# darksim33/Pyneapple

Hardware: AMD Instinct MI355X
Metric: voxels/sec (pixelwise triexp LM & 250-bin NNLS) at 1/2/4/8 MI355X (higher is better)
Workload: dtype f64

## Files before the change

### pyneapple_amd/csrc/pnx_curvefit_kernel.hpp

```cpp
#pragma once
#include <hip/hip_runtime.h>
#include <stdint.h>

namespace pnx {

constexpr int kWave = 64;
constexpr int kMaxB = 128;
constexpr int kMaxP = 8;
#ifdef PNX_ROW_BLK
template <int N> constexpr int row_blk() { return PNX_ROW_BLK; }
#else
template <int N> constexpr int row_blk() { return N >= 7 ? 2 : (N >= 5 ? 4 : 8); }
#endif
constexpr double kEps = 2.220446049250313e-16;
constexpr double kSqrtEps = 1.4901161193847656e-08;
typedef __attribute__((address_space(3))) void lds_void;

struct StreamCtl {
    unsigned long long ready;
    unsigned int abort;
    unsigned int timed_out;
    unsigned int done[1];
};

struct CurvefitArgs {
    const double *y;
    const double *p0;
    const double *lo;
    const double *hi;
    const double *fixed;
    double *popt;
    double *pcov;
    int8_t *status;
    int32_t *nfev;
    double *cost;
    unsigned long long *queue;
    const int32_t *order;
    StreamCtl *ctl;
    unsigned int *host_flags;
    int granule_shift;
    unsigned int stream_spins;
    int phase;
    long long n_vox;
    int n_b;
    int per_voxel;
    int fixed_per_voxel;
    int max_nfev;
    int n_fixed;
    int t1_mode;
    double tr, tm;
    double ftol, xtol, gtol;
    double p0s[kMaxP], los[kMaxP], his[kMaxP], fixeds[kMaxP];
    int free_idx[kMaxP];
    int fixed_idx[kMaxP];
    int use_sigma;
    int absolute_sigma;
    double b[kMaxB];
    double w[kMaxB];
};

template <int MODEL> struct Model;

template <> struct Model<0> {
    static constexpr int NALL = 2, NC = 1;
    __device__ static constexpr int dpos(int c) { return 1; }
    __device__ static double signal(const double *p, const double *E) { return p[0] * E[0]; }
    __device__ static void jac(const double *p, const double *E, double x, double *r) {
        r[0] = E[0];
        r[1] = -x * p[0] * E[0];
    }
};
template <> struct Model<1> {
    static constexpr int NALL = 3, NC = 2;
    __device__ static constexpr int dpos(int c) { return c == 0 ? 1 : 2; }
    __device__ static double signal(const double *p, const double *E) { return p[0] * E[0] + (1 - p[0]) * E[1]; }
    __device__ static void jac(const double *p, const double *E, double x, double *r) {
        r[0] = E[0] - E[1];
        r[1] = -x * p[0] * E[0];
        r[2] = -x * (1 - p[0]) * E[1];
    }
};
template <> struct Model<2> {
    static constexpr int NALL = 4, NC = 2;
    __device__ static constexpr int dpos(int c) { return c == 0 ? 1 : 2; }
    __device__ static double signal(const double *p, const double *E) {
        return p[3] * (p[0] * E[0] + (1 - p[0]) * E[1]);
    }
    __device__ static void jac(const double *p, const double *E, double x, double *r) {
        r[0] = p[3] * (E[0] - E[1]);
        r[1] = -x * p[3] * p[0] * E[0];
        r[2] = -x * p[3] * (1 - p[0]) * E[1];
        r[3] = p[0] * E[0] + (1 - p[0]) * E[1];
    }
};
template <> struct Model<3> {
    static constexpr int NALL = 4, NC = 2;
    __device__ static constexpr int dpos(int c) { return c == 0 ? 1 : 3; }
    __device__ static double signal(const double *p, const double *E) { return p[0] * E[0] + p[2] * E[1]; }
    __device__ static void jac(const double *p, const double *E, double x, double *r) {
        r[0] = E[0];
        r[1] = -x * p[0] * E[0];
        r[2] = E[1];
        r[3] = -x * p[2] * E[1];
    }
};
template <> struct Model<4> {
    static constexpr int NALL = 5, NC = 3;
    __device__ static constexpr int dpos(int c) { return c == 0 ? 1 : (c == 1 ? 3 : 4); }
    __device__ static double signal(const double *p, const double *E) {
        return p[0] * E[0] + p[2] * E[1] + (1 - p[0] - p[2]) * E[2];
    }
    __device__ static void jac(const double *p, const double *E, double x, double *r) {
        const double f3 = 1 - p[0] - p[2];
        r[0] = E[0] - E[2];
        r[1] = -x * p[0] * E[0];
        r[2] = E[1] - E[2];
        r[3] = -x * p[2] * E[1];
        r[4] = -x * f3 * E[2];
    }
};
template <> struct Model<5> {
    static constexpr int NALL = 6, NC = 3;
    __device__ static constexpr int dpos(int c) { return c == 0 ? 1 : (c == 1 ? 3 : 4); }
    __device__ static double signal(const double *p, const double *E) {
        return p[5] * (p[0] * E[0] + p[2] * E[1] + (1 - p[0] - p[2]) * E[2]);
    }
    __device__ static void jac(const double *p, const double *E, double x, double *r) {
        const double f3 = 1 - p[0] - p[2], S0 = p[5];
        r[0] = S0 * (E[0] - E[2]);
        r[1] = -x * S0 * p[0] * E[0];
        r[2] = S0 * (E[1] - E[2]);
        r[3] = -x * S0 * p[2] * E[1];
        r[4] = -x * S0 * f3 * E[2];
        r[5] = p[0] * E[0] + p[2] * E[1] + f3 * E[2];
    }
};
template <> struct Model<6> {
    static constexpr int NALL = 6, NC = 3;
    __device__ static constexpr int dpos(int c) { return c == 0 ? 1 : (c == 1 ? 3 : 5); }
    __device__ static double signal(const double *p, const double *E) {
        return p[0] * E[0] + p[2] * E[1] + p[4] * E[2];
    }
    __device__ static void jac(const double *p, const double *E, double x, double *r) {
        r[0] = E[0];
        r[1] = -x * p[0] * E[0];
        r[2] = E[1];
        r[3] = -x * p[2] * E[1];
        r[4] = E[2];
        r[5] = -x * p[4] * E[2];
    }
};

template <int MODEL> __host__ __device__ constexpr int colperm(int k) {
    constexpr int P[7][6] = {{0, 1, 2, 3, 4, 5}, {2, 0, 1, 3, 4, 5}, {2, 0, 1, 3, 4, 5}, {3, 1, 2, 0, 4, 5},
                             {4, 3, 0, 2, 1, 5}, {4, 3, 0, 2, 1, 5}, {5, 3, 1, 4, 2, 0}};
    return P[MODEL][k];
}

template <int MODEL> __device__ constexpr int comp_of_param(int j) {
    for (int c = 0; c < Model<MODEL>::NC; ++c)
        if (Model<MODEL>::dpos(c) == j) return c;
    return -1;
}

template <int N> __device__ inline double dotn(const double *a, const double *b) {
    double s = 0;
#pragma unroll
    for (int i = 0; i < N; ++i) s += a[i] * b[i];
    return s;
}
template <int N> __device__ inline double normn(const double *a) { return sqrt(dotn<N>(a, a)); }

__device__ inline double fast_rcp(double x) {
    double r = __builtin_amdgcn_rcp(x);
    r = fma(fma(-x, r, 1.0), r, r);
    r = fma(fma(-x, r, 1.0), r, r);
    return r;
}
__device__ inline double fast_sqrt_rsqrt(double x, double *rs) {
    double y = __builtin_amdgcn_rsq(x);
    double g = x * y, h = 0.5 * y;
    double r = fma(-h, g, 0.5);
    g = fma(g, r, g);
    h = fma(h, r, h);
    r = fma(-h, g, 0.5);
    g = fma(g, r, g);
    h = fma(h, r, h);
    *rs = h + h;
    return g;
}

#ifndef PNX_CF_FAST_EXP
#define PNX_CF_FAST_EXP 1
#endif
#ifndef PNX_CF_HINTS
#define PNX_CF_HINTS 1
#endif
#if PNX_CF_HINTS
#define PNX_LIKELY(x) __builtin_expect(!!(x), 1)
#else
#define PNX_LIKELY(x) (x)
#endif
__device__ inline double exp_fast(double x) {
#if PNX_CF_FAST_EXP
    const double k = __builtin_rint(x * 1.4426950408889634);
    double r = fma(k, -0.6931471805599453, x);
    r = fma(k, -2.3190468138462996e-17, r);
    const double r2 = r * r;
    double qe = 2.7630903490112654e-07;
    qe = fma(qe, r2, 2.480149103909504e-05);
    qe = fma(qe, r2, 0.0013888888945916382);
    qe = fma(qe, r2, 0.041666666666519754);
    qe = fma(qe, r2, 0.5000000000000012);
    double qo = 2.502232256764614e-08;
    qo = fma(qo, r2, 2.755751454582531e-06);
    qo = fma(qo, r2, 0.00019841269589115522);
    qo = fma(qo, r2, 0.008333333333455043);
    qo = fma(qo, r2, 0.16666666666666477);
    const double q = fma(r, qo, qe);
    return ldexp(fma(r, fma(r, q, 1.0), 1.0), __double2int_rz(k));
#else
    return exp(x);
#endif
}

template <int N, int RB> __device__ inline void qr_merge(double (&R)[N][N], double (&q)[N], double (&blk)[RB][N + 1]) {
#pragma unroll
    for (int k = 0; k < N; ++k) {
        double sig = 0;
#pragma unroll
        for (int r = 0; r < RB; ++r) sig += blk[r][k] * blk[r][k];
        if (sig > 0) {
            const double alpha = R[k][k];
            double rs;
            const double nrm = fast_sqrt_rsqrt(alpha * alpha + sig, &rs);
            const double beta = alpha <= 0 ? nrm : -nrm;
            const double v0 = alpha - beta;
            const double inv_v0 = copysign(fast_rcp(fabs(v0)), v0);
            const double tau = -v0 * (alpha <= 0 ? rs : -rs);
#pragma unroll
            for (int r = 0; r < RB; ++r) blk[r][k] *= inv_v0;
            R[k][k] = beta;
#pragma unroll
            for (int j = k + 1; j <= N; ++j) {
                double w = (j < N) ? R[k][j] : q[k];
#pragma unroll
                for (int r = 0; r < RB; ++r) w += blk[r][k] * blk[r][j];
                w *= tau;
                if (j < N)
                    R[k][j] -= w;
                else
                    q[k] -= w;
#pragma unroll
                for (int r = 0; r < RB; ++r) blk[r][j] -= w * blk[r][k];
            }
        }
    }
}

template <int N> __device__ inline void jacobi_svd(double (&W)[N][N], double (&V)[N][N]) {
#pragma unroll
    for (int i = 0; i < N; ++i)
#pragma unroll
        for (int j = 0; j < N; ++j) V[i][j] = (i == j) ? 1.0 : 0.0;
    if (N == 1) return;
    for (int sweep = 0; sweep < 30; ++sweep) {
        bool rotated = false;
#pragma unroll
        for (int p = 0; p < N - 1; ++p) {
#pragma unroll
            for (int q = p + 1; q < N; ++q) {
                double a = 0, b = 0, g = 0;
#pragma unroll
                for (int i = 0; i < N; ++i) {
                    a += W[i][p] * W[i][p];
                    b += W[i][q] * W[i][q];
                    g += W[i][p] * W[i][q];
                }
                const double g2 = g * g, ab = a * b;
                if (g2 > 1.0e-30 * ab) {
                    rotated = rotated || (g2 >= 1.0e-16 * ab);
                    const double num = b - a, den = 2.0 * g;
                    double rs;
                    const double hyp = fast_sqrt_rsqrt(num * num + den * den, &rs);
                    double t = fabs(den) * fast_rcp(fabs(num) + hyp);
                    t = ((num < 0) != (den < 0)) ? -t : t;
                    double c;
                    (void)fast_sqrt_rsqrt(1.0 + t * t, &c);
                    const double s = c * t;
#pragma unroll
                    for (int i = 0; i < N; ++i) {
                        const double wp = W[i][p], wq = W[i][q];
                        W[i][p] = c * wp - s * wq;
                        W[i][q] = s * wp + c * wq;
                        const double vp = V[i][p], vq = V[i][q];
                        V[i][p] = c * vp - s * vq;
                        V[i][q] = s * vp + c * vq;
                    }
                }
            }
        }
        if (!rotated) break;
    }
}

__device__ inline double strictly_feasible0(double x, double lb, double ub) {
    if (x <= lb) x = nextafter(lb, ub);
    if (x >= ub) x = nextafter(ub, lb);
    if (x < lb || x > ub) x = 0.5 * (lb + ub);
    return x;
}
__device__ inline double strictly_feasible_r(double x, double lb, double ub) {
    const double rstep = 1e-10;
    const double lower_dist = x - lb, upper_dist = ub - x;
    const double lt = rstep * fmax(1.0, fabs(lb)), ut = rstep * fmax(1.0, fabs(ub));
    int active = 0;
    if (isfinite(lb) && lower_dist <= fmin(upper_dist, lt)) active = -1;
    if (isfinite(ub) && upper_dist <= fmin(lower_dist, ut)) active = 1;
    if (active == -1) x = lb + lt;
    if (active == 1) x = ub - ut;
    if (x < lb || x > ub) x = 0.5 * (lb + ub);
    return x;
}

template <int N>
__device__ inline double step_size_to_bound(const double *x, const double *s, const double *lb, const double *ub,
                                            int *hits) {
    double steps[N];
    double mn = INFINITY;
#pragma unroll
    for (int i = 0; i < N; ++i) {
        const double num = (s[i] > 0) ? (ub[i] - x[i]) : (lb[i] - x[i]);
        steps[i] = (s[i] != 0) ? num / s[i] : INFINITY;
        mn = fmin(mn, steps[i]);
    }
    if (hits) {
#pragma unroll
        for (int i = 0; i < N; ++i) hits[i] = (steps[i] == mn) ? ((s[i] > 0) - (s[i] < 0)) : 0;
    }
    return mn;
}

template <int N> __device__ inline void rmul(const double (&R)[N][N], const double *s, double *out) {
#pragma unroll
    for (int i = 0; i < N; ++i) {
        double a = 0;
#pragma unroll
        for (int j = i; j < N; ++j) a += R[i][j] * s[j];
        out[i] = a;
    }
}

__device__ inline double minimize_quadratic_1d(double a, double b, double lb, double ub, double c, double &y) {
    double tb = lb, yb = lb * (a * lb + b) + c;
    const double yu = ub * (a * ub + b) + c;
    if (yu < yb) {
        yb = yu;
        tb = ub;
    }
    if (a != 0) {
        const double ext = -0.5 * b / a;
        if (lb < ext && ext < ub) {
            const double ye = ext * (a * ext + b) + c;
            if (ye < yb) {
                yb = ye;
                tb = ext;
            }
        }
    }
    y = yb;
    return tb;
}

template <int N>
__device__ inline double solve_lsq_trust_region(int m, const double *uf, const double *s, const double (&V)[N][N],
                                                double smax, double smin, double Delta, double initial_alpha,
                                                double *p) {
    double suf[N], t[N];
#pragma unroll
    for (int i = 0; i < N; ++i) suf[i] = s[i] * uf[i];
    const bool full_rank = (m >= N) && (smin > kEps * m * smax);
    if (full_rank) {
#pragma unroll
        for (int i = 0; i < N; ++i) t[i] = uf[i] / s[i];
#pragma unroll
        for (int i = 0; i < N; ++i) {
            double a = 0;
#pragma unroll
            for (int k = 0; k < N; ++k) a += V[i][k] * t[k];
            p[i] = -a;
        }
        if (normn<N>(p) <= Delta) return 0.0;
    }
    double alpha_upper = normn<N>(suf) / Delta;
    double alpha_lower = 0.0;
    auto phi_and_derivative = [&](double alpha, double &phi, double &phi_prime) {
        double pn2 = 0, sp = 0;
#pragma unroll
        for (int i = 0; i < N; ++i) {
            const double denom = s[i] * s[i] + alpha;
            const double q = suf[i] / denom;
            pn2 += q * q;
            sp += suf[i] * suf[i] / (denom * denom * denom);
        }
        const double p_norm = sqrt(pn2);
        phi = p_norm - Delta;
        phi_prime = -sp / p_norm;
    };
    double phi, phi_prime;
    if (full_rank) {
        phi_and_derivative(0.0, phi, phi_prime);
        alpha_lower = -phi / phi_prime;
    }
    double alpha;
    if (!full_rank && initial_alpha == 0)
        alpha = fmax(0.001 * alpha_upper, sqrt(alpha_lower * alpha_upper));
    else
        alpha = initial_alpha;
    for (int it = 0; it < 10; ++it) {
        if (alpha < alpha_lower || alpha > alpha_upper)
            alpha = fmax(0.001 * alpha_upper, sqrt(alpha_lower * alpha_upper));
        phi_and_derivative(alpha, phi, phi_prime);
        if (phi < 0) alpha_upper = alpha;
        const double ratio = phi / phi_prime;
        alpha_lower = fmax(alpha_lower, alpha - ratio);
        alpha -= (phi + Delta) * ratio / Delta;
        if (fabs(phi) < 0.01 * Delta) break;
    }
#pragma unroll
    for (int i = 0; i < N; ++i) t[i] = suf[i] / (s[i] * s[i] + alpha);
#pragma unroll
    for (int i = 0; i < N; ++i) {
        double a = 0;
#pragma unroll
        for (int k = 0; k < N; ++k) a += V[i][k] * t[k];
        p[i] = -a;
    }
    const double sc = Delta / normn<N>(p);
#pragma unroll
    for (int i = 0; i < N; ++i) p[i] *= sc;
    return alpha;
}

template <int N>
__device__ inline double select_step(const double *x, const double (&R2)[N][N], const double *g_h, double *p,
                                     double *p_h, const double *d, double Delta, const double *lb, const double *ub,
                                     double theta, double *step, double *step_h) {
    bool inb = true;
#pragma unroll
    for (int i = 0; i < N; ++i) {
        const double xp = x[i] + p[i];
        inb = inb && (xp >= lb[i]) && (xp <= ub[i]);
    }
    double t1[N], t2[N];
    if (inb) {
        rmul<N>(R2, p_h, t1);
        const double p_value = 0.5 * dotn<N>(t1, t1) + dotn<N>(p_h, g_h);
#pragma unroll
        for (int i = 0; i < N; ++i) {
            step[i] = p[i];
            step_h[i] = p_h[i];
        }
        return -p_value;
    }
    int hits[N];
    const double p_stride = step_size_to_bound<N>(x, p, lb, ub, hits);
    double r_h[N], r[N], xb[N];
#pragma unroll
    for (int i = 0; i < N; ++i) {
        r_h[i] = hits[i] ? -p_h[i] : p_h[i];
        r[i] = d[i] * r_h[i];
    }
#pragma unroll
    for (int i = 0; i < N; ++i) {
        p[i] *= p_stride;
        p_h[i] *= p_stride;
        xb[i] = x[i] + p[i];
    }
    double to_tr;
    {
        const double a = dotn<N>(r_h, r_h), b = dotn<N>(p_h, r_h), c = dotn<N>(p_h, p_h) - Delta * Delta;
        const double dd = sqrt(b * b - a * c);
        const double q = -(b + copysign(dd, b));
        const double ta = q / a, tb = c / q;
        to_tr = fmax(ta, tb);
    }
    double to_bound = step_size_to_bound<N>(xb, r, lb, ub, nullptr);
    double r_stride = fmin(to_bound, to_tr);
    double r_stride_l, r_stride_u;
    if (r_stride > 0) {
        r_stride_l = (1 - theta) * p_stride / r_stride;
        r_stride_u = (r_stride == to_bound) ? theta * to_bound : to_tr;
    } else {
        r_stride_l = 0;
        r_stride_u = -1;
    }
    double r_value;
    if (r_stride_l <= r_stride_u) {
        rmul<N>(R2, r_h, t1);
        rmul<N>(R2, p_h, t2);
        const double a = 0.5 * dotn<N>(t1, t1);
        const double b = dotn<N>(g_h, r_h) + dotn<N>(t2, t1);
        const double c = 0.5 * dotn<N>(t2, t2) + dotn<N>(g_h, p_h);
        r_stride = minimize_quadratic_1d(a, b, r_stride_l, r_stride_u, c, r_value);
#pragma unroll
        for (int i = 0; i < N; ++i) {
            r_h[i] = r_h[i] * r_stride + p_h[i];
            r[i] = r_h[i] * d[i];
        }
    } else
        r_value = INFINITY;
#pragma unroll
    for (int i = 0; i < N; ++i) {
        p[i] *= theta;
        p_h[i] *= theta;
    }
    rmul<N>(R2, p_h, t1);
    const double p_value = 0.5 * dotn<N>(t1, t1) + dotn<N>(p_h, g_h);

    double ag_h[N], ag[N];
#pragma unroll
    for (int i = 0; i < N; ++i) {
        ag_h[i] = -g_h[i];
        ag[i] = d[i] * ag_h[i];
    }
    to_tr = Delta / normn<N>(ag_h);
    to_bound = step_size_to_bound<N>(x, ag, lb, ub, nullptr);
    double ag_stride = (to_bound < to_tr) ? theta * to_bound : to_tr;
    double ag_value;
    {
        rmul<N>(R2, ag_h, t1);
        const double a = 0.5 * dotn<N>(t1, t1);
        const double b = dotn<N>(g_h, ag_h);
        ag_stride = minimize_quadratic_1d(a, b, 0.0, ag_stride, 0.0, ag_value);
    }
    if (p_value < r_value && p_value < ag_value) {
#pragma unroll
        for (int i = 0; i < N; ++i) {
            step[i] = p[i];
            step_h[i] = p_h[i];
        }
        return -p_value;
    } else if (r_value < p_value && r_value < ag_value) {
#pragma unroll
        for (int i = 0; i < N; ++i) {
            step[i] = r[i];
            step_h[i] = r_h[i];
        }
        return -r_value;
    } else {
#pragma unroll
        for (int i = 0; i < N; ++i) {
            step[i] = ag[i] * ag_stride;
            step_h[i] = ag_h[i] * ag_stride;
        }
        return -ag_value;
    }
}

enum LaneState : int { ST_IDLE = 0, ST_INIT = 1, ST_RUN = 2, ST_FINAL = 3 };

template <int N> struct Park {
    static constexpr int NR = N * (N + 1) / 2;
    static constexpr bool kParkV = (N <= 5);
    static constexpr int NV = kParkV ? N * N : 0;
    __host__ __device__ static constexpr int per_wave(int n_b) { return kWave * (((n_b + 1) & ~1) + NR + NV); }
};

#ifndef PNX_CF_WAVES_PER_SIMD
#define PNX_CF_WAVES_PER_SIMD 1
#endif
#ifndef PNX_CF_BLOCK_WAVES
#define PNX_CF_BLOCK_WAVES 4
#endif
template <int MODEL, int N, bool FD, bool PV, bool T1, bool STREAM = false>
__global__ void __launch_bounds__(64 * PNX_CF_BLOCK_WAVES, PNX_CF_WAVES_PER_SIMD) curvefit_kernel(const CurvefitArgs A) {
    using M = Model<MODEL>;
    using PK = Park<N>;
    constexpr int NALL = M::NALL;
    constexpr int NP = NALL + (T1 ? 1 : 0);
    constexpr int NC = M::NC;
    constexpr bool HASFIXED = (N != NP);
    static_assert(!(FD && HASFIXED), "finite-difference mode is only built without fixed parameters");
    auto CP = [](int k) constexpr { return (HASFIXED || k >= NALL) ? k : colperm<MODEL>(k); };

    extern __shared__ double smem[];
    const int n_b = A.n_b;
    double *bsh = smem;
    const int lane = threadIdx.x & (kWave - 1);
    const int wave = threadIdx.x / kWave;
    const bool use_w = A.use_sigma != 0;
    const double *wsh = smem + kMaxB;
    double *ytile = smem + (use_w ? 2 * kMaxB : kMaxB) + (size_t)wave * PK::per_wave(n_b);
    double *ysh = ytile + 2 * lane;
    double *rpark = ytile + (size_t)((n_b + 1) & ~1) * kWave + lane;
    double *vpark = rpark + (size_t)PK::NR * kWave;
    for (int i = threadIdx.x; i < n_b; i += blockDim.x) bsh[i] = A.b[i];
    if (use_w)
        for (int i = threadIdx.x; i < n_b; i += blockDim.x) smem[kMaxB + i] = A.w[i];
    __syncthreads();
    const bool dma_ok = ((reinterpret_cast<uintptr_t>(A.y) & 7) == 0);

    int state = ST_IDLE;
    long long vox = -1;
    unsigned long long ready_seen = 0;
    int pub = 0;
    auto publish = [&](bool all) {
        const int n_gran = (int)((A.n_vox + (1ll << A.granule_shift) - 1) >> A.granule_shift);
        int upto = pub;
        while (upto < n_gran && (all || !__ballot(state != ST_IDLE && (vox >> A.granule_shift) <= upto))) ++upto;
        if (upto == pub) return;
        __builtin_amdgcn_fence(__ATOMIC_RELEASE, "");
        const unsigned int n_waves = gridDim.x * (blockDim.x / kWave);
        if ((threadIdx.x & (kWave - 1)) == __ffsll((unsigned long long)__ballot(1)) - 1) {
            for (int g = pub; g < upto; ++g) {
                const unsigned int old = __hip_atomic_fetch_add(&A.ctl->done[g], 1u, __ATOMIC_ACQ_REL, __HIP_MEMORY_SCOPE_SYSTEM);
                if (old + 1 == n_waves) __hip_atomic_store(&A.host_flags[g], 1u, __ATOMIC_RELEASE, __HIP_MEMORY_SCOPE_SYSTEM);
            }
        }
        pub = upto;
    };
    double x[N], lb[N], ub[N];
    double pfull[NP];
    double g[N];
    double s[N], uf[N], R2[N][N], d[N], g_h[N];
    double Vreg[PK::kParkV ? 1 : N][PK::kParkV ? 1 : N];
    double smax = 0, smin = 0, theta = 0;
    double cost = 0, Delta = 0, alpha = 0;
    int nfev = 0, term = -99;
    bool first = false;
    double xn[N], step_h_norm = 0, step_norm = 0, predicted = 0;
    if (!PV) {
#pragma unroll
        for (int k = 0; k < N; ++k) {
            lb[k] = A.los[k];
            ub[k] = A.his[k];
        }
    }

#ifdef PNX_CF_STAMP
    unsigned long long seg[8] = {0, 0, 0, 0, 0, 0, 0, 0}, act[8] = {0, 0, 0, 0, 0, 0, 0, 0}, cnt[8] = {0, 0, 0, 0, 0, 0, 0, 0};
    unsigned long long tl = __builtin_amdgcn_s_memtime();
#define CFSTAMP(k) do { __builtin_amdgcn_s_waitcnt(0); const unsigned long long t_ = __builtin_amdgcn_s_memtime(); seg[k] += t_ - tl; tl = t_; } while (0)
#define CFACT(k, cond) do { act[k] += __popcll(__ballot(cond)); cnt[k] += 1; } while (0)
#else
#define CFSTAMP(k) do {} while (0)
#define CFACT(k, cond) do {} while (0)
#endif
    auto refill = [&]() {
    while (state == ST_IDLE) {
        const unsigned long long idx = atomicAdd(A.queue, 1ULL);
        if (idx >= (unsigned long long)A.n_vox) break;
        if constexpr (STREAM) {
            if (idx >= ready_seen) {
                bool got = false;
                const unsigned int *abort_word = A.host_flags + ((A.n_vox + (1ll << A.granule_shift) - 1) >> A.granule_shift);
                for (unsigned int spins = 0; spins < A.stream_spins; ++spins) {
                    ready_seen = __hip_atomic_load(&A.ctl->ready, __ATOMIC_ACQUIRE, __HIP_MEMORY_SCOPE_SYSTEM);
                    if (idx < ready_seen) {
                        got = true;
                        break;
                    }
                    if ((spins & 15u) == 15u && __hip_atomic_load(abort_word, __ATOMIC_RELAXED, __HIP_MEMORY_SCOPE_SYSTEM)) break;
                    __builtin_amdgcn_s_sleep(127);
                }
                if (!got) {
                    if (!__hip_atomic_load(abort_word, __ATOMIC_RELAXED, __HIP_MEMORY_SCOPE_SYSTEM))
                        __hip_atomic_store(&A.ctl->timed_out, 1u, __ATOMIC_RELAXED, __HIP_MEMORY_SCOPE_SYSTEM);
                    break;
                }
            }
        }
        vox = (long long)idx;
        if constexpr (!STREAM) {
            if (A.order) vox = A.order[idx];
        }
        const double *yv = A.y + (size_t)vox * n_b;
        if (dma_ok) {
            const int pairs = n_b >> 1;
            for (int c = 0; c < pairs; ++c)
                __builtin_amdgcn_global_load_lds((const void *)(yv + 2 * c), (lds_void *)(ytile + c * 2 * kWave), 16, 0, 0);
            if (n_b & 1) {
                if (vox + 1 < A.n_vox)
                    __builtin_amdgcn_global_load_lds((const void *)(yv + n_b - 1), (lds_void *)(ytile + pairs * 2 * kWave), 16, 0, 0);
                else
                    ysh[pairs * 2 * kWave] = yv[n_b - 1];
            }
        } else {
            for (int i = 0; i < n_b; ++i) ysh[(i >> 1) * 2 * kWave + (i & 1)] = yv[i];
        }
        bool okb = true, okp = true;
        double p0v[N];
#pragma unroll
        for (int k = 0; k < N; ++k) {
            if (PV) {
                p0v[k] = A.p0[(size_t)k * A.n_vox + vox];
                lb[k] = A.lo[(size_t)k * A.n_vox + vox];
                ub[k] = A.hi[(size_t)k * A.n_vox + vox];
            } else
                p0v[k] = A.p0s[k];
            okb = okb && (lb[k] < ub[k]);
            okp = okp && (p0v[k] >= lb[k]) && (p0v[k] <= ub[k]);
        }
        if (HASFIXED) {
#pragma unroll
            for (int j = 0; j < NP; ++j) pfull[j] = 0;
            for (int f = 0; f < A.n_fixed; ++f) {
                const double fv = A.fixed_per_voxel ? A.fixed[(size_t)f * A.n_vox + vox] : A.fixeds[f];
#pragma unroll
                for (int j = 0; j < NP; ++j)
                    if (A.fixed_idx[f] == j) pfull[j] = fv;
            }
        }
        if (!okb || !okp) {
            const int st = !okb ? -1 : -3;
#pragma unroll
            for (int k = 0; k < N; ++k) A.popt[(size_t)k * A.n_vox + vox] = p0v[k];
            if (A.status) A.status[vox] = (int8_t)st;
            if (A.nfev) A.nfev[vox] = 0;
            if (A.cost) A.cost[vox] = NAN;
            continue;
        }
#pragma unroll
        for (int k = 0; k < N; ++k) xn[k] = strictly_feasible_r(p0v[k], lb[k], ub[k]);
        state = ST_INIT;
        nfev = 0;
        term = -99;
        alpha = 0.0;
    }
    };
    refill();
    if constexpr (STREAM) {
        if (!__ballot(state != ST_IDLE)) publish(true);
    }
    for (;;) {
        CFSTAMP(7);
        if (state == ST_IDLE) break;
        asm volatile("s_waitcnt vmcnt(0)" ::: "memory");
        CFSTAMP(0);
        CFACT(1, true);

        double Rn[N][N], qn[N], gn[N], cost_new = 0;
        bool finite_f = true, yfinite = true;
        {
            double pe[NP];
            if (HASFIXED) {
#pragma unroll
                for (int j = 0; j < NP; ++j) {
                    pe[j] = pfull[j];
#pragma unroll
                    for (int k = 0; k < N; ++k)
                        if (A.free_idx[k] == j) pe[j] = xn[k];
                }
            } else {
#pragma unroll
                for (int j = 0; j < NP; ++j) pe[j] = xn[j];
            }
            double dxv[N];
            if (FD) {
#pragma unroll
                for (int k = 0; k < N; ++k) {
                    const double sign = (xn[k] >= 0) ? 1.0 : -1.0;
                    double h = kSqrtEps * sign * fmax(1.0, fabs(xn[k]));
                    const double lower_dist = xn[k] - lb[k], upper_dist = ub[k] - xn[k];
                    const double xx = xn[k] + h;
                    const bool violated = (xx < lb[k]) || (xx > ub[k]);
                    const bool fitting = fabs(h) <= fmax(lower_dist, upper_dist);
                    if (violated && fitting) h = -h;
                    if (!fitting) h = (upper_dist >= lower_dist) ? upper_dist : -lower_dist;
                    dxv[k] = (xn[k] + h) - xn[k];
                }
            }
            double A1 = 1.0, eTM = 1.0, fac = 1.0, dfac = 0.0;
            if (T1) {
                const bool steam = A.t1_mode == 2;
                const double T1v = pe[NALL];
                const double eTR = exp(-A.tr / T1v);
                A1 = 1 - eTR;
                eTM = steam ? exp(-A.tm / T1v) : 1.0;
                fac = A1 * eTM;
                dfac = steam ? eTM / (T1v * T1v) * (-A.tr * eTR + A.tm * A1) : (-eTR * A.tr / (T1v * T1v));
                if (FD) {
                    const double dx = dxv[N - 1];
                    const double T2 = T1v + dx;
                    const double fac2 = (1 - exp(-A.tr / T2)) * (steam ? exp(-A.tm / T2) : 1.0);
                    dfac = (fac2 - fac) / dx;
                }
            }
#pragma unroll
            for (int i = 0; i < N; ++i) {
                qn[i] = 0;
                gn[i] = 0;
#pragma unroll
                for (int j = 0; j < N; ++j) Rn[i][j] = 0;
            }
            constexpr int kRowBlk = row_blk<N>();
            for (int i0 = 0; i0 < n_b; i0 += kRowBlk) {
                double blk[kRowBlk][N + 1];
#pragma unroll
                for (int r = 0; r < kRowBlk; ++r) {
                    const int i = i0 + r;
                    const bool live = i < n_b;
                    const int ii = live ? i : 0;
                    const double bb = bsh[ii];
                    const double nb = -bb;
                    const double yi = ysh[(ii >> 1) * 2 * kWave + (ii & 1)];
                    yfinite = yfinite && isfinite(yi);
                    double E[NC];
#pragma unroll
                    for (int c = 0; c < NC; ++c) E[c] = exp_fast(nb * pe[M::dpos(c)]);
                    const double base = M::signal(pe, E);
                    double r0 = (T1 ? base * A1 * eTM : base) - yi;
                    double jr[N];
                    {
                        double ja[NP];
                        M::jac(pe, E, bb, ja);
                        if (FD) {
#pragma unroll
                            for (int k = 0; k < NALL; ++k) {
                                if (comp_of_param<MODEL>(k) >= 0) {
                                    const double z = nb * dxv[k];
                                    double gz;
#if PNX_CF_FAST_EXP
                                    if (PNX_LIKELY(fabs(z) < 2e-4))
                                        gz = fma(z, fma(z, fma(z, 1.0 / 24, 1.0 / 6), 0.5), 1.0);
                                    else
#endif
                                    if (fabs(z) < 1e-3)
                                        gz = 1.0 + z * (0.5 + z * (1.0 / 6 + z * (1.0 / 24 + z * (1.0 / 120 + z * (1.0 / 720)))));
                                    else
                                        gz = expm1(z) / z;
                                    ja[k] *= gz;
                                }
                            }
                        }
                        if (T1) {
#pragma unroll
                            for (int k = 0; k < NALL; ++k) ja[k] *= fac;
                            ja[NP - 1] = base * dfac;
                        }
                        if (use_w) {
                            const double t = wsh[ii];
                            r0 *= t;
#pragma unroll
                            for (int k = 0; k < NP; ++k) ja[k] *= t;
                        }
                        if (HASFIXED) {
#pragma unroll
                            for (int k = 0; k < N; ++k) {
                                jr[k] = 0;
#pragma unroll
                                for (int j = 0; j < NP; ++j)
                                    if (A.free_idx[k] == j) jr[k] = ja[j];
                            }
                        } else {
#pragma unroll
                            for (int k = 0; k < N; ++k) jr[k] = ja[k];
                        }
                    }
                    const double rr = live ? r0 : 0.0;
                    finite_f = finite_f && isfinite(rr);
                    cost_new += rr * rr;
#pragma unroll
                    for (int k = 0; k < N; ++k) {
                        const double jk = live ? jr[k] : 0.0;
                        gn[k] += jk * rr;
                    }
#pragma unroll
                    for (int k = 0; k < N; ++k) blk[r][k] = live ? jr[CP(k)] : 0.0;
                    blk[r][N] = rr;
                }
                CFSTAMP(1);
                qr_merge<N, kRowBlk>(Rn, qn, blk);
                CFSTAMP(6);
            }
            cost_new *= 0.5;
        }

        CFSTAMP(1);
        bool accepted = false;
        int final_status = 0;
        if (state == ST_INIT) {
            if (!finite_f) {
                final_status = yfinite ? -4 : -2;
                cost = NAN;
                nfev = 0;
                state = ST_FINAL;
            } else {
                accepted = true;
                nfev = 1;
                first = true;
                state = ST_RUN;
            }
        } else {
            nfev += 1;
            if (!finite_f) {
                Delta = 0.25 * step_h_norm;
            } else {
                const double actual = cost - cost_new;
                double ratio;
                if (predicted > 0)
                    ratio = actual / predicted;
                else if (predicted == 0 && actual == 0)
                    ratio = 1;
                else
                    ratio = 0;
                double Delta_new = Delta;
                if (ratio < 0.25)
                    Delta_new = 0.25 * step_h_norm;
                else if (ratio > 0.75 && step_h_norm > 0.95 * Delta)
                    Delta_new = Delta * 2.0;
                const bool ftol_ok = (actual < A.ftol * cost) && (ratio > 0.25);
                const bool xtol_ok = step_norm < A.xtol * (A.xtol + normn<N>(x));
                if (ftol_ok && xtol_ok)
                    term = 4;
                else if (ftol_ok)
                    term = 2;
                else if (xtol_ok)
                    term = 3;
                if (term == -99) {
                    alpha *= Delta / Delta_new;
                    Delta = Delta_new;
                }
                accepted = actual > 0;
            }
        }
        if (accepted) {
#pragma unroll
            for (int i = 0; i < N; ++i) {
                x[i] = xn[i];
                g[i] = gn[i];
            }
            cost = cost_new;
            int t = 0;
#pragma unroll
            for (int i = 0; i < N; ++i)
#pragma unroll
                for (int j = i; j < N; ++j) rpark[(t++) * kWave] = Rn[i][j];
        }

        double v[N], dv[N], g_norm = 0;
        if (state == ST_RUN && (accepted || term != -99 || nfev >= A.max_nfev)) {
#pragma unroll
            for (int i = 0; i < N; ++i) {
                v[i] = 1.0;
                dv[i] = 0.0;
                if (g[i] < 0 && isfinite(ub[i])) {
                    v[i] = ub[i] - x[i];
                    dv[i] = -1;
                }
                if (g[i] > 0 && isfinite(lb[i])) {
                    v[i] = x[i] - lb[i];
                    dv[i] = 1;
                }
                g_norm = fmax(g_norm, fabs(g[i] * v[i]));
            }
            if (first) {
                double t = 0;
#pragma unroll
                for (int i = 0; i < N; ++i) {
                    const double q = x[i] / sqrt(v[i]);
                    t += q * q;
                }
                Delta = sqrt(t);
                if (Delta == 0) Delta = 1.0;
                first = false;
            }
            if (g_norm < A.gtol) term = 1;
            if (term != -99 || nfev >= A.max_nfev) {
                final_status = (term == -99) ? 0 : term;
                state = ST_FINAL;
            }
        }

        CFSTAMP(2);
        CFACT(3, state == ST_FINAL);
        if (state == ST_FINAL) {
            const bool ok = final_status > 0;
#pragma unroll
            for (int k = 0; k < N; ++k) {
                const double pk = ok ? x[k] : (PV ? A.p0[(size_t)k * A.n_vox + vox] : A.p0s[k]);
                A.popt[(size_t)k * A.n_vox + vox] = pk;
            }
            if (A.status) A.status[vox] = (int8_t)final_status;
            if (A.nfev) A.nfev[vox] = nfev;
            if (A.cost) A.cost[vox] = cost;
            if (A.pcov && ok) {
                double *pc = A.pcov + (size_t)vox * N * N;
#pragma unroll
                for (int t = 0; t < PK::NR; ++t) pc[t] = rpark[t * kWave];
            }
            state = ST_IDLE;
        }
        CFACT(0, state == ST_IDLE);
        if constexpr (STREAM) {
            const bool any_idle = __ballot(state == ST_IDLE) != 0;
            if (state == ST_IDLE) refill();
            if (any_idle) publish(false);
        } else {
            if (state == ST_IDLE) refill();
        }

        CFSTAMP(3);
        CFACT(4, state == ST_RUN && accepted);
        CFACT(5, state == ST_RUN);
        if (state == ST_RUN) {
            if (accepted) {
                double diag_h[N];
#pragma unroll
                for (int i = 0; i < N; ++i) {
                    d[i] = sqrt(v[i]);
                    diag_h[i] = g[i] * dv[i];
                    g_h[i] = d[i] * g[i];
                }
                double q2[N];
                double blk[N][N + 1];
#pragma unroll
                for (int i = 0; i < N; ++i) {
                    q2[i] = qn[i];
#pragma unroll
                    for (int j = 0; j < N; ++j) {
                        R2[i][j] = (j >= i) ? Rn[i][j] * d[CP(j)] : 0.0;
                        blk[i][j] = (i == j) ? sqrt(diag_h[CP(i)]) : 0.0;
                    }
                    blk[i][N] = 0.0;
                }
                qr_merge<N, N>(R2, q2, blk);
                double W[N][N], Vw[N][N];
#pragma unroll
                for (int i = 0; i < N; ++i)
#pragma unroll
                    for (int j = 0; j < N; ++j) W[i][j] = (i >= j) ? R2[j][i] : 0.0;
                jacobi_svd<N>(W, Vw);
                smax = 0;
                smin = INFINITY;
#pragma unroll
                for (int k = 0; k < N; ++k) {
                    double nn = 0, dq = 0;
#pragma unroll
                    for (int i = 0; i < N; ++i) {
                        nn += W[i][k] * W[i][k];
                        dq += Vw[i][k] * q2[i];
                    }
                    double inv = 0.0;
                    if (nn > 0) nn = fast_sqrt_rsqrt(nn, &inv);
                    s[k] = nn;
                    uf[k] = dq;
#pragma unroll
                    for (int i = 0; i < N; ++i) {
                        if (PK::kParkV)
                            vpark[(i * N + k) * kWave] = W[i][k] * inv;
                        else
                            Vreg[PK::kParkV ? 0 : i][PK::kParkV ? 0 : k] = W[i][k] * inv;
                    }
                    smax = fmax(smax, nn);
                    smin = fmin(smin, nn);
                }
                theta = fmax(0.995, 1 - g_norm);
            }
            CFSTAMP(4);
            double V[N][N];
#pragma unroll
            for (int i = 0; i < N; ++i)
#pragma unroll
                for (int k = 0; k < N; ++k)
                    V[i][k] = PK::kParkV ? vpark[(i * N + k) * kWave] : Vreg[PK::kParkV ? 0 : i][PK::kParkV ? 0 : k];
            double xP[N], lbP[N], ubP[N], dP[N], ghP[N];
#pragma unroll
            for (int i = 0; i < N; ++i) {
                xP[i] = x[CP(i)];
                lbP[i] = lb[CP(i)];
                ubP[i] = ub[CP(i)];
                dP[i] = d[CP(i)];
                ghP[i] = g_h[CP(i)];
            }
            double p_h[N], p[N], step[N], step_h[N];
            alpha = solve_lsq_trust_region<N>(n_b, uf, s, V, smax, smin, Delta, alpha, p_h);
#pragma unroll
            for (int i = 0; i < N; ++i) p[i] = dP[i] * p_h[i];
            predicted = select_step<N>(xP, R2, ghP, p, p_h, dP, Delta, lbP, ubP, theta, step, step_h);
#pragma unroll
            for (int i = 0; i < N; ++i) xn[CP(i)] = strictly_feasible0(xP[i] + step[i], lbP[i], ubP[i]);
            step_h_norm = normn<N>(step_h);
            step_norm = normn<N>(step);
            CFSTAMP(5);
        }
    }
#ifdef PNX_CF_STAMP
    if (threadIdx.x == 0 && blockIdx.x == 3)
        printf("CFSTAMP refill=%llu pass_rows=%llu pass_qr_merge=%llu D+Blight=%llu final=%llu Bheavy=%llu C=%llu loop=%llu | iters=%llu idle_at_top=%.2f final=%.2f Bheavy=%.2f run=%.2f\n",
               seg[0], seg[1], seg[6], seg[2], seg[3], seg[4], seg[5], seg[7], cnt[1], (double)act[0] / cnt[0], (double)act[3] / cnt[3],
               (double)act[4] / cnt[4], (double)act[5] / cnt[5]);
#endif
}

struct ColPerm {
    int p[kMaxP];
};

template <int N>
__global__ void __launch_bounds__(256) pcov_kernel(double *pcov, const int8_t *status, const double *cost,
                                                   long long n_vox, int n_b, const ColPerm cp, int absolute_sigma) {
    const long long vox = (long long)blockIdx.x * blockDim.x + threadIdx.x;
    if (vox >= n_vox) return;
    double *pc = pcov + (size_t)vox * N * N;
    if (status[vox] <= 0) {
#pragma unroll
        for (int k = 0; k < N * N; ++k) pc[k] = NAN;
        return;
    }
    double W[N][N], Vw[N][N];
    {
        int t = 0;
#pragma unroll
        for (int i = 0; i < N; ++i)
#pragma unroll
            for (int j = 0; j < N; ++j) W[i][j] = 0.0;
#pragma unroll
        for (int i = 0; i < N; ++i)
#pragma unroll
            for (int j = i; j < N; ++j) W[j][i] = pc[t++];
    }
    jacobi_svd<N>(W, Vw);
    double s2[N], sm = 0;
#pragma unroll
    for (int k = 0; k < N; ++k) {
        double nn = 0;
#pragma unroll
        for (int i = 0; i < N; ++i) nn += W[i][k] * W[i][k];
        s2[k] = nn;
        sm = fmax(sm, nn);
    }
    const double thr = kEps * (n_b > N ? n_b : N) * sqrt(sm);
    const bool dof = absolute_sigma || n_b > N;
    const double s_sq = absolute_sigma ? 1.0 : (dof ? 2.0 * cost[vox] / (double)(n_b - N) : 0.0);
    double wgt[N];
#pragma unroll
    for (int k = 0; k < N; ++k) wgt[k] = (sqrt(s2[k]) > thr) ? 1.0 / (s2[k] * s2[k]) : 0.0;
    bool bad = false;
    double out[N][N];
#pragma unroll
    for (int i = 0; i < N; ++i)
#pragma unroll
        for (int j = 0; j < N; ++j) {
            double a = 0;
#pragma unroll
            for (int k = 0; k < N; ++k) a += W[i][k] * W[j][k] * wgt[k];
            out[i][j] = a;
            bad = bad || isnan(a);
        }
#pragma unroll
    for (int i = 0; i < N; ++i)
#pragma unroll
        for (int j = 0; j < N; ++j) pc[cp.p[i] * N + cp.p[j]] = (bad || !dof) ? INFINITY : out[i][j] * s_sq;
}

}
```

Before: 112.8 million.

## Specialize curve-fit row loop by tail, weights, and uniform fast-gz range

```diff
diff --git a/pyneapple_amd/csrc/pnx_curvefit_kernel.hpp b/pyneapple_amd/csrc/pnx_curvefit_kernel.hpp
--- a/pyneapple_amd/csrc/pnx_curvefit_kernel.hpp
+++ b/pyneapple_amd/csrc/pnx_curvefit_kernel.hpp
@@ -14,6 +14,9 @@
 #endif
 constexpr double kEps = 2.220446049250313e-16;
 constexpr double kSqrtEps = 1.4901161193847656e-08;
+template <bool B> struct BoolC {
+    static constexpr bool value = B;
+};
 typedef __attribute__((address_space(3))) void lds_void;
 
 struct StreamCtl {
@@ -598,6 +601,11 @@
     for (int i = threadIdx.x; i < n_b; i += blockDim.x) bsh[i] = A.b[i];
     if (use_w)
         for (int i = threadIdx.x; i < n_b; i += blockDim.x) smem[kMaxB + i] = A.w[i];
+    double bmax = 0;
+    for (int i = 0; i < n_b; ++i) {
+        const double ab = fabs(A.b[i]);
+        bmax = (ab < INFINITY) ? fmax(bmax, ab) : INFINITY;
+    }
     __syncthreads();
     const bool dma_ok = ((reinterpret_cast<uintptr_t>(A.y) & 7) == 0);
 
@@ -795,16 +803,29 @@
                 for (int j = 0; j < N; ++j) Rn[i][j] = 0;
             }
             constexpr int kRowBlk = row_blk<N>();
-            for (int i0 = 0; i0 < n_b; i0 += kRowBlk) {
+            static_assert(kRowBlk % 2 == 0, "a block reads its signal values as [pair][lane][2] pairs");
+            auto row_block = [&](auto fastgz_c, auto usew_c, auto tail_c, const int i0) __attribute__((always_inline)) {
+                constexpr bool FASTGZ = decltype(fastgz_c)::value, USEW = decltype(usew_c)::value, TAIL = decltype(tail_c)::value;
                 double blk[kRowBlk][N + 1];
+                double bv[TAIL ? 1 : kRowBlk], yv[TAIL ? 1 : kRowBlk];
+                if constexpr (!TAIL) {
+#pragma unroll
+                    for (int r = 0; r < kRowBlk; r += 2) {
+                        const double2 b2 = *reinterpret_cast<const double2 *>(bsh + i0 + r);
+                        const double2 y2 = *reinterpret_cast<const double2 *>(ysh + (size_t)(i0 + r) * kWave);
+                        bv[r] = b2.x;
+                        bv[r + 1] = b2.y;
+                        yv[r] = y2.x;
+                        yv[r + 1] = y2.y;
+                    }
+                }
 #pragma unroll
                 for (int r = 0; r < kRowBlk; ++r) {
-                    const int i = i0 + r;
-                    const bool live = i < n_b;
-                    const int ii = live ? i : 0;
-                    const double bb = bsh[ii];
+                    const bool live = !TAIL || (i0 + r < n_b);
+                    const int ii = live ? i0 + r : 0;
+                    const double bb = TAIL ? bsh[ii] : bv[TAIL ? 0 : r];
                     const double nb = -bb;
-                    const double yi = ysh[(ii >> 1) * 2 * kWave + (ii & 1)];
+                    const double yi = TAIL ? ysh[(ii >> 1) * 2 * kWave + (ii & 1)] : yv[TAIL ? 0 : r];
                     yfinite = yfinite && isfinite(yi);
                     double E[NC];
 #pragma unroll
@@ -822,7 +843,7 @@
                                     const double z = nb * dxv[k];
                                     double gz;
 #if PNX_CF_FAST_EXP
-                                    if (PNX_LIKELY(fabs(z) < 2e-4))
+                                    if (FASTGZ || PNX_LIKELY(fabs(z) < 2e-4))
                                         gz = fma(z, fma(z, fma(z, 1.0 / 24, 1.0 / 6), 0.5), 1.0);
                                     else
 #endif
@@ -839,7 +860,7 @@
                             for (int k = 0; k < NALL; ++k) ja[k] *= fac;
                             ja[NP - 1] = base * dfac;
                         }
-                        if (use_w) {
+                        if (TAIL ? use_w : USEW) {
                             const double t = wsh[ii];
                             r0 *= t;
 #pragma unroll
@@ -873,6 +894,32 @@
                 CFSTAMP(1);
                 qr_merge<N, kRowBlk>(Rn, qn, blk);
                 CFSTAMP(6);
+            };
+            auto row_loop = [&](auto fastgz_c, auto usew_c) __attribute__((always_inline)) {
+                int i0 = 0;
+                for (; i0 + kRowBlk <= n_b; i0 += kRowBlk) row_block(fastgz_c, usew_c, BoolC<false>{}, i0);
+                if (i0 < n_b) row_block(BoolC<false>{}, BoolC<false>{}, BoolC<true>{}, i0);
+            };
+            constexpr bool kOneLoop = (N >= 6);
+            bool gz_cubic = FD && PNX_CF_FAST_EXP && !kOneLoop;
+            if (FD && PNX_CF_FAST_EXP && !kOneLoop) {
+                bool in_range = true;
+#pragma unroll
+                for (int k = 0; k < NALL; ++k)
+                    if (comp_of_param<MODEL>(k) >= 0) in_range = in_range && (fabs(bmax * dxv[k]) < 2e-4);
+                gz_cubic = __ballot(!in_range) == 0;
+            }
+            if constexpr (kOneLoop) {
+                for (int i0 = 0; i0 < n_b; i0 += kRowBlk) row_block(BoolC<false>{}, BoolC<false>{}, BoolC<true>{}, i0);
+            } else if (PNX_LIKELY(!use_w && (gz_cubic || !FD))) {
+                if constexpr (FD && PNX_CF_FAST_EXP)
+                    row_loop(BoolC<true>{}, BoolC<false>{});
+                else
+                    row_loop(BoolC<false>{}, BoolC<false>{});
+            } else if (use_w) {
+                row_loop(BoolC<false>{}, BoolC<true>{});
+            } else {
+                if constexpr (FD) row_loop(BoolC<false>{}, BoolC<false>{});
             }
             cost_new *= 0.5;
         }
```

After: 128.2 million (median of 6 runs). +13.6%, better.
